# rongzhao-zhang/EfficientQ

Hardware: AMD Instinct MI355X
Metric: ptq_calibration_throughput (higher is better)
Workload: dtype i8xi8->i32 (exact) for the Gram systems and per-iteration loss convs of the layers with quantised input, f32/f64 elsewhere

## Files before the change

efficientq_amd/csrc/prox_solve.hip:

```cpp
#include "common.h"
#include "internal.h"
#include "project_dual.h"

namespace effq {

typedef float f32x16 __attribute__((ext_vector_type(16)));
typedef float f32x4 __attribute__((ext_vector_type(4)));

__global__ __launch_bounds__(256) void k_build_b(const float* __restrict__ B0, const float* __restrict__ W0,
                                                 const float* __restrict__ b0, const float* __restrict__ G,
                                                 const float* __restrict__ dual, int c2, int n, int has_bias,
                                                 float rho, float eta, float* __restrict__ Bm, int ldb, int c2p,
                                                 const float* __restrict__ wprev, float shift) {
  const size_t tot = (size_t)c2p * ldb;
  const size_t stride = (size_t)gridDim.x * blockDim.x;
  const int nw = n - has_bias;
  for (size_t e = (size_t)blockIdx.x * blockDim.x + threadIdx.x; e < tot; e += stride) {
    const int r = (int)(e / ldb), k = (int)(e % ldb);
    float v = 0.0f;
    if (r < c2 && k < n) {
      if (k < nw) {
        const size_t wi = (size_t)r * nw + k;
        v = prox_rhs(B0[(size_t)r * n + k], W0[wi], G[wi], dual[wi], eta, rho);
        if (wprev != nullptr) v = v + shift * wprev[wi];
      } else {
        v = B0[(size_t)r * n + k] + eta * b0[r];
      }
    }
    Bm[e] = v;
  }
}

__global__ __launch_bounds__(256) void k_build_b4(const float* __restrict__ B0, const float* __restrict__ W0,
                                                  const float* __restrict__ b0, const float* __restrict__ G,
                                                  const float* __restrict__ dual, int c2, int n, int has_bias,
                                                  float rho, float eta, float* __restrict__ Bm, int ldb,
                                                  const float* __restrict__ wprev, float shift) {
  __builtin_amdgcn_s_setprio(2);

  const int r = blockIdx.y;
  const int nw = n - has_bias;
  float* out = Bm + (size_t)r * ldb;
  for (int k = (blockIdx.x * blockDim.x + threadIdx.x) * 4; k < ldb; k += gridDim.x * blockDim.x * 4) {
    float4 v = make_float4(0.f, 0.f, 0.f, 0.f);
    if (r < c2 && k < nw) {
      const size_t wi = (size_t)r * nw + k;
      const float* bp = B0 + (size_t)r * n + k;
      const float4 w0 = *reinterpret_cast<const float4*>(W0 + wi), g = *reinterpret_cast<const float4*>(G + wi),
                   du = *reinterpret_cast<const float4*>(dual + wi);
      v.x = prox_rhs(bp[0], w0.x, g.x, du.x, eta, rho);
      v.y = prox_rhs(bp[1], w0.y, g.y, du.y, eta, rho);
      v.z = prox_rhs(bp[2], w0.z, g.z, du.z, eta, rho);
      v.w = prox_rhs(bp[3], w0.w, g.w, du.w, eta, rho);
      if (wprev != nullptr) {
        const float4 wp = *reinterpret_cast<const float4*>(wprev + wi);
        v.x = v.x + shift * wp.x;
        v.y = v.y + shift * wp.y;
        v.z = v.z + shift * wp.z;
        v.w = v.w + shift * wp.w;
      }
    } else if (r < c2 && k == nw && has_bias) {
      v.x = B0[(size_t)r * n + k] + eta * b0[r];
    }
    *reinterpret_cast<float4*>(out + k) = v;
  }
}

__global__ __launch_bounds__(256) void k_prox_reduce4(const float* __restrict__ part, int ldp, int nsplit, int c2, int n,
                                                      int has_bias, float* __restrict__ wstar, float* __restrict__ bstar) {
  __builtin_amdgcn_s_setprio(2);

  const int r = blockIdx.y;
  const int nw = n - has_bias;
  const size_t tot = (size_t)c2 * ldp;
  const float* row = part + (size_t)r * ldp;
  for (int k = (blockIdx.x * blockDim.x + threadIdx.x) * 4; k < ldp; k += gridDim.x * blockDim.x * 4) {
    if (k >= n) continue;
    float4 v = *reinterpret_cast<const float4*>(row + k);
    for (int z = 1; z < nsplit; ++z) {
      const float4 t = *reinterpret_cast<const float4*>(row + (size_t)z * tot + k);
      v.x += t.x;
      v.y += t.y;
      v.z += t.z;
      v.w += t.w;
    }
    if (k < nw)
      *reinterpret_cast<float4*>(wstar + (size_t)r * nw + k) = v;
    else
      bstar[r] = v.x;
  }
}

constexpr int PBK = 32, PLD = PBK + 4;

template <int MT, int WM, int WN, int NTN>
__global__ __launch_bounds__(256) void k_prox_gemm(const float* __restrict__ Bm, int ldb, const float* __restrict__ Ainv,
                                                   int lda, int n, int c2, int has_bias, float* __restrict__ wstar,
                                                   float* __restrict__ bstar, float* __restrict__ part, int ldp) {
  __builtin_amdgcn_s_setprio(2);

  constexpr int BM = 32 * MT * WM, BN = 32 * WN * NTN;
  constexpr int NA = BM * 8 / 256, NB = BN * 8 / 256;
  static_assert(WM * WN == 4 && NA >= 1 && NB >= 1, "4 waves");
  __shared__ __attribute__((aligned(16))) float As[BM * PLD];
  __shared__ __attribute__((aligned(16))) float Bs[BN * PLD];
  const int tid = threadIdx.x, lane = tid & 63, wid = tid >> 6;
  const int li = lane & 31, lh = lane >> 5;
  const int wm = wid / WN, wn = wid % WN;
  const int row0 = blockIdx.y * BM, col0 = blockIdx.x * BN;

  f32x16 acc[MT][NTN];
#pragma unroll
  for (int m = 0; m < MT; ++m)
#pragma unroll
    for (int t = 0; t < NTN; ++t)
#pragma unroll
      for (int r = 0; r < 16; ++r) acc[m][t][r] = 0.0f;

  f32x4 ra[NA], rb[NB];
  const float* pa[NA];
  const float* pb[NB];
#pragma unroll
  for (int q = 0; q < NA; ++q) {
    const int u = tid + q * 256, r = u >> 3, c4 = u & 7;
    pa[q] = Bm + (size_t)(row0 + r) * ldb + c4 * 4;
  }
#pragma unroll
  for (int q = 0; q < NB; ++q) {
    const int u = tid + q * 256, r = u >> 3, c4 = u & 7;
    pb[q] = Ainv + (size_t)min(col0 + r, n - 1) * lda + c4 * 4;
  }
#define EFFQ_PROX_FETCH(k0)                                                         \
  {                                                                                 \
    _Pragma("unroll") for (int q = 0; q < NA; ++q)                                  \
        ra[q] = *reinterpret_cast<const f32x4*>(pa[q] + (k0));                      \
    _Pragma("unroll") for (int q = 0; q < NB; ++q)                                  \
        rb[q] = *reinterpret_cast<const f32x4*>(pb[q] + (k0));                      \
  }
  const int nkt = ldb / PBK;
  const int kt0 = (int)(((long long)nkt * blockIdx.z) / gridDim.z);
  const int nk = (int)(((long long)nkt * (blockIdx.z + 1)) / gridDim.z);
  EFFQ_PROX_FETCH(kt0 * PBK)
  for (int kt = kt0; kt < nk; ++kt) {
    lds_barrier();
#pragma unroll
    for (int q = 0; q < NA; ++q) {
      const int u = tid + q * 256;
      *reinterpret_cast<f32x4*>(&As[(u >> 3) * PLD + (u & 7) * 4]) = ra[q];
    }
#pragma unroll
    for (int q = 0; q < NB; ++q) {
      const int u = tid + q * 256;
      *reinterpret_cast<f32x4*>(&Bs[(u >> 3) * PLD + (u & 7) * 4]) = rb[q];
    }
    lds_barrier();
    EFFQ_PROX_FETCH(min(kt + 1, nk - 1) * PBK)
    __builtin_amdgcn_sched_barrier(0);
#pragma unroll
    for (int q = 0; q < 4; ++q) {
      f32x4 a[MT], b[NTN];
#pragma unroll
      for (int m = 0; m < MT; ++m)
        a[m] = *reinterpret_cast<const f32x4*>(&As[((wm * MT + m) * 32 + li) * PLD + q * 8 + 4 * lh]);
#pragma unroll
      for (int t = 0; t < NTN; ++t)
        b[t] = *reinterpret_cast<const f32x4*>(&Bs[((wn * NTN + t) * 32 + li) * PLD + q * 8 + 4 * lh]);
#pragma unroll
      for (int m = 0; m < MT; ++m)
#pragma unroll
        for (int t = 0; t < NTN; ++t)
#pragma unroll
          for (int e = 0; e < 4; ++e)
            acc[m][t] = __builtin_amdgcn_mfma_f32_32x32x2f32(a[m][e], b[t][e], acc[m][t], 0, 0, 0);
    }
  }
#undef EFFQ_PROX_FETCH
  const int nw = n - has_bias;
  if (gridDim.z > 1) {
    float* P = part + (size_t)blockIdx.z * c2 * ldp;
#pragma unroll
    for (int m = 0; m < MT; ++m)
#pragma unroll
      for (int t = 0; t < NTN; ++t) {
        const int col = col0 + (wn * NTN + t) * 32 + li;
#pragma unroll
        for (int r = 0; r < 16; ++r) {
          const int row = row0 + (wm * MT + m) * 32 + (r & 3) + 8 * (r >> 2) + 4 * lh;
          if (row < c2 && col < n) P[(size_t)row * ldp + col] = acc[m][t][r];
        }
      }
    return;
  }
#pragma unroll
  for (int m = 0; m < MT; ++m)
#pragma unroll
    for (int t = 0; t < NTN; ++t) {
      const int col = col0 + (wn * NTN + t) * 32 + li;
#pragma unroll
      for (int r = 0; r < 16; ++r) {
        const int row = row0 + (wm * MT + m) * 32 + (r & 3) + 8 * (r >> 2) + 4 * lh;
        if (row < c2 && col < n) {
          if (col < nw)
            wstar[(size_t)row * nw + col] = acc[m][t][r];
          else
            bstar[row] = acc[m][t][r];
        }
      }
    }
}


typedef __bf16 bf16x8 __attribute__((ext_vector_type(8)));
typedef __bf16 bf16x4 __attribute__((ext_vector_type(4)));
constexpr int B3_K = 16;
constexpr int B3_LD = B3_K + 8;

__device__ __forceinline__ void split3(const f32x4 v, bf16x4& p0, bf16x4& p1, bf16x4& p2) {
#pragma unroll
  for (int e = 0; e < 4; ++e) {
    const __bf16 b0 = (__bf16)v[e];
    const float r1 = v[e] - (float)b0;
    const __bf16 b1 = (__bf16)r1;
    const float r2 = r1 - (float)b1;
    p0[e] = b0;
    p1[e] = b1;
    p2[e] = (__bf16)r2;
  }
}

template <int BM, int BN, int WM, int WN>
__global__ __launch_bounds__(512) void k_prox_gemm_b3(const float* __restrict__ Bm, int ldb, const float* __restrict__ Ainv,
                                                      int lda, int n, int c2, int has_bias, float* __restrict__ wstar,
                                                      float* __restrict__ bstar, float* __restrict__ part, int ldp) {
  __builtin_amdgcn_s_setprio(2);
  constexpr int MT = BM / WM / 32, NT = BN / WN / 32;
  constexpr int NA = BM * 4 / 512, NB = BN * 4 / 512;
  constexpr int STAGE = 3 * (BM + BN) * B3_LD;
  static_assert(WM * WN == 8 && MT >= 1 && NT >= 1 && NA >= 1 && NB >= 1, "8 waves");
  extern __shared__ __attribute__((aligned(16))) unsigned char b3_lds[];
  __bf16* lds = reinterpret_cast<__bf16*>(b3_lds);
  const int tid = threadIdx.x, lane = tid & 63, wid = tid >> 6;
  const int li = lane & 31, lh = lane >> 5;
  const int wm = wid / WN, wn = wid % WN;
  const int row0 = blockIdx.y * BM, col0 = blockIdx.x * BN;

// ... 101 lines not shown
          else if (col < nw)
            wstar[(size_t)row * nw + col] = acc[m][t][r];
          else
            bstar[row] = acc[m][t][r];
        }
      }
    }
}

__global__ __launch_bounds__(256) void k_prox_reduce(const float* __restrict__ part, int ldp, int nsplit, int c2, int n,
                                                     int has_bias, float* __restrict__ wstar, float* __restrict__ bstar) {
  const size_t tot = (size_t)c2 * ldp, stride = (size_t)gridDim.x * blockDim.x;
  const int nw = n - has_bias;
  for (size_t e = (size_t)blockIdx.x * blockDim.x + threadIdx.x; e < tot; e += stride) {
    const int row = (int)(e / ldp), col = (int)(e % ldp);
    if (col >= n) continue;
    float v = part[e];
    for (int z = 1; z < nsplit; ++z) v += part[(size_t)z * tot + e];
    if (col < nw)
      wstar[(size_t)row * nw + col] = v;
    else
      bstar[row] = v;
  }
}

enum ProxVariant { PROX_F32_256 = 0, PROX_F32_128 = 1, PROX_F32_64 = 2, PROX_F32_32 = 3, PROX_B3_256 = 5, PROX_B3_128 = 7 };
typedef void (*ProxGemm)(const float*, int, const float*, int, int, int, int, float*, float*, float*, int);
struct ProxTile {
  ProxVariant variant;
  int bm, bn, threads;
  size_t lds;
  ProxGemm kernel;
  hipError_t (*raise_lds)(size_t);
};
template <int MT, int WM, int WN, int NTN>
static ProxTile f32_tile(ProxVariant v) {
  return ProxTile{v, 32 * MT * WM, 32 * WN * NTN, 256, 0, k_prox_gemm<MT, WM, WN, NTN>, nullptr};
}
template <int BM, int BN, int WM, int WN>
static ProxTile b3_tile(ProxVariant v) {
  return ProxTile{v, BM, BN, 512, (size_t)2 * 3 * (BM + BN) * B3_LD * sizeof(__bf16), k_prox_gemm_b3<BM, BN, WM, WN>,
                  raise_lds_limit<k_prox_gemm_b3<BM, BN, WM, WN>>};
}
static const ProxTile TILE_F32_256 = f32_tile<2, 4, 1, 2>(PROX_F32_256);
static const ProxTile TILE_F32_128 = f32_tile<1, 4, 1, 2>(PROX_F32_128);
static const ProxTile TILE_F32_64 = f32_tile<1, 2, 2, 1>(PROX_F32_64);
static const ProxTile TILE_F32_32 = f32_tile<1, 1, 4, 1>(PROX_F32_32);
static const ProxTile TILE_B3_256 = b3_tile<256, 256, 4, 2>(PROX_B3_256);
static const ProxTile TILE_B3_128 = b3_tile<128, 128, 2, 4>(PROX_B3_128);

struct ProxPlan {
  const ProxTile* tile;
  int gx, gy, nsplit, c2p, ldb;
};
static ProxPlan prox_plan(int c2, int n) {
  ProxPlan p;
  p.c2p = (c2 > 128) ? round_up(c2, 256) : (c2 > 64) ? 128 : round_up(c2, 32);
  p.ldb = round_up(n, 32);
  const bool b3 = p.c2p >= 128 && n >= 1024;
  if (b3) p.tile = (p.c2p == 128) ? &TILE_B3_128 : &TILE_B3_256;
  else p.tile = (p.c2p >= 256) ? &TILE_F32_256 : (p.c2p == 128) ? &TILE_F32_128 : (p.c2p == 64) ? &TILE_F32_64 : &TILE_F32_32;
  p.gx = (n + p.tile->bn - 1) / p.tile->bn;
  p.gy = p.c2p / p.tile->bm;
  const int tiles = p.gx * p.gy;
  if (b3) {
    const int nkt5 = p.ldb / B3_K;
    int s5 = (256 + tiles / 2) / tiles;
    if (s5 > nkt5 / 16) s5 = nkt5 / 16;
    if (s5 < 1) s5 = 1;
    p.nsplit = s5;
    return p;
  }
  const int nkt = p.ldb / PBK;
  int s = (440 + tiles - 1) / tiles;
  if (s > nkt / 6) s = nkt / 6;
  if (s > 16) s = 16;
  if (s < 1) s = 1;
  if (p.tile == &TILE_F32_256) {
    const int smax = s > 1 ? 16 : 1;
    double best = -1.0;
    for (int c = 1; c <= smax && c <= nkt / 6; ++c) {
      const int wgs = tiles * c, rounds = (wgs + 767) / 768;
      const double score = (double)wgs / (768.0 * rounds) - 0.01 * c;
      if (score > best) { best = score; s = c; }
    }
  }
  p.nsplit = s;
  return p;
}

}

using namespace effq;

extern "C" {

int effq_prox_plan_query(int c2, int n, int* variant, int* gx, int* gy, int* nsplit) {
  EFFQ_CHECK_ARG(c2 > 0 && n > 0 && variant && gx && gy && nsplit);
  const ProxPlan p = prox_plan(c2, n);
  *variant = p.tile->variant;
  *gx = p.gx;
  *gy = p.gy;
  *nsplit = p.nsplit;
  return EFFQ_OK;
}

size_t effq_prox_ws_bytes(int c2, int n) {
  if (c2 <= 0 || n <= 0) return 0;
  const ProxPlan p = prox_plan(c2, n);
  return ((size_t)p.c2p + (p.nsplit > 1 ? (size_t)p.nsplit * c2 : 0)) * p.ldb * sizeof(float) + 256;
}

static int launch_build(const ProxSolve& s, const ProxPlan& pl, float* Bm, const float* wprev, hipStream_t st) {
  const int hb = s.has_bias ? 1 : 0;
  if (((s.n - hb) % 4) == 0) {
    const unsigned bx = (unsigned)((pl.ldb / 4 + 255) / 256);
    hipLaunchKernelGGL(k_build_b4, dim3(bx, (unsigned)pl.c2p), dim3(256), 0, st, s.B0, s.W0, s.b0, s.G, s.dual, s.c2, s.n,
                       hb, (float)s.rho, (float)s.eta, Bm, pl.ldb, wprev, (float)s.shift);
  } else {
    size_t nb = ((size_t)pl.c2p * pl.ldb + 255) / 256;
    if (nb > 4096) nb = 4096;
    hipLaunchKernelGGL(k_build_b, dim3((unsigned)nb), dim3(256), 0, st, s.B0, s.W0, s.b0, s.G, s.dual, s.c2, s.n, hb,
                       (float)s.rho, (float)s.eta, Bm, pl.ldb, pl.c2p, wprev, (float)s.shift);
  }
  EFFQ_LAUNCH_CHECK();
  return EFFQ_OK;
}

static int launch_gemm(const ProxSolve& s, const ProxPlan& pl, const float* Bm, float* part, hipStream_t st) {
  const ProxTile& t = *pl.tile;
  if (t.lds > 0) EFFQ_HIP(t.raise_lds(t.lds));
  hipLaunchKernelGGL(t.kernel, dim3(pl.gx, pl.gy, pl.nsplit), dim3(t.threads), t.lds, st, Bm, pl.ldb, s.Ainv,
                     effq_ainv_ld(s.n), s.n, s.c2, s.has_bias ? 1 : 0, s.wstar, s.bstar, part, pl.ldb);
  EFFQ_LAUNCH_CHECK();
  return EFFQ_OK;
}

static int launch_reduce(const ProxSolve& s, const ProxPlan& pl, const float* part, hipStream_t st) {
  const int hb = s.has_bias ? 1 : 0;
  if (((s.n - hb) % 4) == 0) {
    const unsigned bx = (unsigned)((pl.ldb / 4 + 255) / 256);
    hipLaunchKernelGGL(k_prox_reduce4, dim3(bx, (unsigned)s.c2), dim3(256), 0, st, part, pl.ldb, pl.nsplit, s.c2, s.n, hb,
                       s.wstar, s.bstar);
  } else {
    size_t nb = ((size_t)s.c2 * pl.ldb + 255) / 256;
    if (nb > 2048) nb = 2048;
    hipLaunchKernelGGL(k_prox_reduce, dim3((unsigned)nb), dim3(256), 0, st, part, pl.ldb, pl.nsplit, s.c2, s.n, hb,
                       s.wstar, s.bstar);
  }
  EFFQ_LAUNCH_CHECK();
  return EFFQ_OK;
}

int effq_prox_enqueue(const ProxSolve* sp, void* stream) {
  EFFQ_CHECK_ARG(sp != nullptr);
  const ProxSolve& s = *sp;
  EFFQ_CHECK_ARG(s.B0 && s.Ainv && s.W0 && s.G && s.dual && s.wstar && s.ws && s.c2 > 0 && s.n > 0 && s.nterms >= 1);
  EFFQ_CHECK_ARG(!s.has_bias || (s.b0 != nullptr && s.bstar != nullptr));
  if (s.ws_bytes < effq_prox_ws_bytes(s.c2, s.n)) {
    set_error("prox_solve: workspace %zu < required %zu", s.ws_bytes, effq_prox_ws_bytes(s.c2, s.n));
    return EFFQ_ERR_WORKSPACE;
  }
  const ProxPlan pl = prox_plan(s.c2, s.n);
  float* Bm = reinterpret_cast<float*>(s.ws);
  float* part = Bm + (size_t)pl.c2p * pl.ldb;
  hipStream_t st = as_stream(stream);
  for (int term = 0; term < s.nterms; ++term) {
    if (!(s.prebuilt && term == 0))
      if (const int rc = launch_build(s, pl, Bm, (term > 0) ? s.wstar : nullptr, st); rc != EFFQ_OK) return rc;
    if (const int rc = launch_gemm(s, pl, Bm, part, st); rc != EFFQ_OK) return rc;
    if (s.parts != nullptr)
      *s.parts = ProxParts{(pl.nsplit > 1) ? part : nullptr, pl.nsplit, pl.ldb};
    else if (pl.nsplit > 1)
      if (const int rc = launch_reduce(s, pl, part, st); rc != EFFQ_OK) return rc;
  }
  return EFFQ_OK;
}

int effq_prox_solve(const float* B0, const float* Ainv, const float* W0, const float* b0, const float* G,
                    const float* dual, int c2, int n, int has_bias, double rho, double eta, float* wstar, float* bstar,
                    void* ws, size_t ws_bytes, void* stream) {
  const ProxSolve s = {B0, Ainv, W0, b0, G, dual, c2, n, has_bias, rho, eta, 0.0, 1, false, wstar, bstar, ws, ws_bytes,
                       nullptr};
  return effq_prox_enqueue(&s, stream);
}

int effq_prox_solve_shifted(const float* B0, const float* Ainv, const float* W0, const float* b0, const float* G,
                            const float* dual, int c2, int n, int has_bias, double rho, double eta, double rho_inv,
                            int nterms, float* wstar, float* bstar, void* ws, size_t ws_bytes, void* stream) {
  EFFQ_CHECK_ARG(rho_inv >= rho && rho > 0.0 && eta >= 0.0);
  const ProxSolve s = {B0, Ainv, W0, b0, G, dual, c2, n, has_bias, rho, eta, rho_inv - rho, nterms, false, wstar, bstar,
                       ws, ws_bytes, nullptr};
  return effq_prox_enqueue(&s, stream);
}

float* effq_prox_bm(void* ws, int c2, int n, int* ldb) {
  *ldb = prox_plan(c2, n).ldb;
  return reinterpret_cast<float*>(ws);
}

}
```

efficientq_amd/csrc/spd_inverse.hip:

```cpp
#include <vector>
#include "common.h"

namespace effq {

typedef double f64x4 __attribute__((ext_vector_type(4)));

constexpr int NBK = 64;
constexpr int LDA_S = 66;
constexpr int LDB_S = 80;

__global__ __launch_bounds__(256) void k_build_a64(const float* __restrict__ A0, int n, int npad, int has_bias,
                                                   double rho, double eta, double* __restrict__ A64) {
  const size_t tot = (size_t)npad * npad;
  const size_t stride = (size_t)gridDim.x * blockDim.x;
  for (size_t e = (size_t)blockIdx.x * blockDim.x + threadIdx.x; e < tot; e += stride) {
    const int i = (int)(e / npad), j = (int)(e % npad);
    double v = 0.0;
    if (i < n && j < n) {
      v = (double)A0[(size_t)i * n + j];
      if (i == j) v += eta + ((has_bias && i == n - 1) ? 0.0 : rho);
    } else if (i == j) {
      v = 1.0;
    }
    A64[e] = v;
  }
}

__device__ __forceinline__ double readlane_f64(double v, int lane) {
  const int lo = __builtin_amdgcn_readlane(__double2loint(v), lane);
  const int hi = __builtin_amdgcn_readlane(__double2hiint(v), lane);
  return __hiloint2double(hi, lo);
}

template <int CPW>
__device__ __forceinline__ void gj_invert_regs(double (&reg)[CPW], double (*fcol)[NBK + 1], int lane, int wid) {
#pragma unroll
  for (int p = 0; p < NBK; ++p) {
    const int par = p & 1, wp = p / CPW, jp = p % CPW;
    if (wid == wp) {
      double cp = reg[0];
#pragma unroll
      for (int j = 1; j < CPW; ++j) cp = (jp == j) ? reg[j] : cp;
      fcol[par][lane] = cp;
      if (lane == p) fcol[par][NBK] = 1.0 / cp;
    }
    lds_barrier();
    const double piv = fcol[par][NBK];
    const double f = fcol[par][lane];
#pragma unroll
    for (int j = 0; j < CPW; ++j) {
      const double rp = readlane_f64(reg[j], p) * piv;
      const bool colp = (wid == wp) && (jp == j);
      double v;
      if (lane == p)
        v = colp ? piv : rp;
      else
        v = colp ? (-f * piv) : (reg[j] - f * rp);
      reg[j] = v;
    }
  }
}

constexpr int GJD_T = 1024, GJD_CPW = NBK / (GJD_T / 64);
__global__ __launch_bounds__(GJD_T) void k_gj_diag(const double* __restrict__ A, int npad, int kb,
                                                   double* __restrict__ Dinv) {
  __shared__ double fcol[2][NBK + 1];
  const int lane = threadIdx.x & 63, wid = threadIdx.x >> 6;
  double reg[GJD_CPW];
#pragma unroll
  for (int j = 0; j < GJD_CPW; ++j) reg[j] = A[(size_t)(kb + lane) * npad + kb + wid * GJD_CPW + j];
  gj_invert_regs<GJD_CPW>(reg, fcol, lane, wid);
#pragma unroll
  for (int j = 0; j < GJD_CPW; ++j) Dinv[lane * NBK + wid * GJD_CPW + j] = reg[j];
}

__device__ __forceinline__ void tile_mma64(const double* As, const double* Bs, f64x4 (&acc)[2][2]) {
  const int lane = threadIdx.x & 63, wid = threadIdx.x >> 6;
  const int wr = wid >> 1, wc = wid & 1;
  const int lr = lane & 15, lk = lane >> 4;
#pragma unroll 4
  for (int ks = 0; ks < NBK / 4; ++ks) {
    double a[2], b[2];
#pragma unroll
    for (int mi = 0; mi < 2; ++mi) a[mi] = As[(wr * 32 + mi * 16 + lr) * LDA_S + ks * 4 + lk];
#pragma unroll
    for (int ni = 0; ni < 2; ++ni) b[ni] = Bs[(ks * 4 + lk) * LDB_S + wc * 32 + ni * 16 + lr];
#pragma unroll
    for (int mi = 0; mi < 2; ++mi)
#pragma unroll
      for (int ni = 0; ni < 2; ++ni) acc[mi][ni] = __builtin_amdgcn_mfma_f64_16x16x4f64(a[mi], b[ni], acc[mi][ni], 0, 0, 0);
  }
}

__device__ __forceinline__ void load_tile(double* dst, int ld, const double* src, size_t src_ld) {
  const int tid = threadIdx.x;
  for (int e = tid; e < NBK * NBK; e += 256) {
    const int r = e >> 6, c = e & 63;
    dst[r * ld + c] = src[(size_t)r * src_ld + c];
  }
}

constexpr int GJ_CT = 4;

__global__ __launch_bounds__(256) void k_gj_panel(double* __restrict__ A, int npad, int kb,
                                                  const double* __restrict__ Dinv, double* __restrict__ NZ,
                                                  double* __restrict__ XT) {
  extern __shared__ __attribute__((aligned(16))) double sm[];
  double* As = sm;
  double* Bs = sm + NBK * LDA_S;
  const int kblk = kb / NBK;
  const int t = blockIdx.x;
  const int tid = threadIdx.x, lane = tid & 63, wid = tid >> 6;
  const int wr = wid >> 1, wc = wid & 1;
  if (t == kblk) {
    for (int e = tid; e < NBK * NBK; e += 256) A[(size_t)(kb + (e >> 6)) * npad + kb + (e & 63)] = Dinv[e];
    return;
  }
  const bool upper = t < kblk;
  const double sgn = upper ? -1.0 : 1.0;
  for (int e = tid; e < NBK * NBK; e += 256) {
    const int r = e >> 6, c = e & 63;
    const double v = upper ? A[(size_t)(t * NBK + r) * npad + kb + c] : A[(size_t)(kb + r) * npad + (size_t)t * NBK + c];
    if (upper) {
      As[r * LDA_S + c] = v;
    } else {
      As[c * LDA_S + r] = v;
    }
  }
  load_tile(Bs, LDB_S, Dinv, NBK);
  lds_barrier();
  for (int e = tid; e < NBK * NBK; e += 256) {
    const int kk = e >> 6, r = e & 63;
    XT[(size_t)kk * npad + (size_t)t * NBK + r] = sgn * As[r * LDA_S + kk];
  }
  f64x4 acc[2][2];
#pragma unroll
  for (int mi = 0; mi < 2; ++mi)
#pragma unroll
    for (int ni = 0; ni < 2; ++ni)
#pragma unroll
      for (int r = 0; r < 4; ++r) acc[mi][ni][r] = 0.0;
  tile_mma64(As, Bs, acc);
  const int lr = lane & 15, lk = lane >> 4;
#pragma unroll
  for (int mi = 0; mi < 2; ++mi)
#pragma unroll
    for (int ni = 0; ni < 2; ++ni)
#pragma unroll
      for (int r = 0; r < 4; ++r) {
        const int row = wr * 32 + mi * 16 + lk + 4 * r;
        const int col = wc * 32 + ni * 16 + lr;
        const double z = acc[mi][ni][r];
        NZ[(size_t)(t * NBK + row) * NBK + col] = -z;
        if (upper)
          A[(size_t)(t * NBK + row) * npad + kb + col] = -z;
        else
          A[(size_t)(kb + col) * npad + (size_t)t * NBK + row] = z;
      }
}

__global__ __launch_bounds__(256) void k_gj_trail_sym(double* __restrict__ A, int npad, int kb,
                                                      const double* __restrict__ NZ, const double* __restrict__ XT,
                                                      double* __restrict__ Dinv_next) {
  __shared__ __attribute__((aligned(16))) double As[NBK * LDA_S];
  __shared__ double fcol[2][NBK + 1];
  const int kblk = kb / NBK, nblk = npad / NBK;
  const int kn = kblk + 1;
  const bool ahead = Dinv_next != nullptr && kn < nblk;
  const int tid = threadIdx.x, lane = tid & 63, wid = tid >> 6;
  const int wr = wid >> 1, wc = wid & 1;
  const int lr = lane & 15, lk = lane >> 4;
  if (blockIdx.y == 0) {
    if (blockIdx.x != 0 || !ahead) return;
    for (int e = tid; e < NBK * NBK; e += 256) {
      const int r = e >> 6, c = e & 63;
      As[r * LDA_S + c] = NZ[(size_t)(kn * NBK + r) * NBK + c];
    }
    lds_barrier();
    const double* Cb = A + (size_t)(kn * NBK + wr * 32) * npad + (size_t)kn * NBK + wc * 32;
    const double* Rb = XT + (size_t)kn * NBK + wc * 32;
    f64x4 acc[2][2];
#pragma unroll
    for (int mi = 0; mi < 2; ++mi)
#pragma unroll
      for (int ni = 0; ni < 2; ++ni)
#pragma unroll
        for (int r = 0; r < 4; ++r) acc[mi][ni][r] = Cb[(size_t)(mi * 16 + lk + 4 * r) * npad + ni * 16 + lr];
#pragma unroll 4
    for (int ks = 0; ks < NBK / 4; ++ks) {
      double a[2], b[2];
#pragma unroll
      for (int mi = 0; mi < 2; ++mi) a[mi] = As[(wr * 32 + mi * 16 + lr) * LDA_S + ks * 4 + lk];
#pragma unroll
      for (int ni = 0; ni < 2; ++ni) b[ni] = Rb[(size_t)(ks * 4 + lk) * npad + ni * 16 + lr];
#pragma unroll
      for (int mi = 0; mi < 2; ++mi)
#pragma unroll
        for (int ni = 0; ni < 2; ++ni) acc[mi][ni] = __builtin_amdgcn_mfma_f64_16x16x4f64(a[mi], b[ni], acc[mi][ni], 0, 0, 0);
    }
    lds_barrier();
#pragma unroll
    for (int mi = 0; mi < 2; ++mi)
#pragma unroll
      for (int ni = 0; ni < 2; ++ni)
#pragma unroll
        for (int r = 0; r < 4; ++r)
          As[(wr * 32 + mi * 16 + lk + 4 * r) * LDA_S + wc * 32 + ni * 16 + lr] = acc[mi][ni][r];
    lds_barrier();
    constexpr int CPW = NBK / 4;
    double reg[CPW];
#pragma unroll
    for (int j = 0; j < CPW; ++j) reg[j] = As[lane * LDA_S + wid * CPW + j];
    gj_invert_regs<CPW>(reg, fcol, lane, wid);
#pragma unroll
    for (int j = 0; j < CPW; ++j) Dinv_next[lane * NBK + wid * CPW + j] = reg[j];
    return;
  }
  const int ib = (int)blockIdx.y - 1;
  if (ib == kblk) return;
  if ((int)(blockIdx.x * GJ_CT + GJ_CT - 1) < ib) return;
  for (int e = tid; e < NBK * NBK; e += 256) {
    const int r = e >> 6, c = e & 63;
    As[r * LDA_S + c] = NZ[(size_t)(ib * NBK + r) * NBK + c];
  }
  lds_barrier();
  auto live = [&](int t) -> bool {
    const int jb = blockIdx.x * GJ_CT + t;
    return t < GJ_CT && jb < nblk && jb != kblk && jb >= ib && !(ahead && ib == kn && jb == kn);
  };
  auto fetch = [&](int t, f64x4 (&c)[2][2]) {
    const int jb = blockIdx.x * GJ_CT + t;
    const double* Cb = A + (size_t)(ib * NBK + wr * 32) * npad + (size_t)jb * NBK + wc * 32;
#pragma unroll
    for (int mi = 0; mi < 2; ++mi)
#pragma unroll
      for (int ni = 0; ni < 2; ++ni)
#pragma unroll
        for (int r = 0; r < 4; ++r) c[mi][ni][r] = Cb[(size_t)(mi * 16 + lk + 4 * r) * npad + ni * 16 + lr];
  };
  f64x4 nxt[2][2];
  int t = 0;
  while (t < GJ_CT && !live(t)) ++t;
  if (t < GJ_CT) fetch(t, nxt);
  while (t < GJ_CT) {
    const int jb = blockIdx.x * GJ_CT + t;
    f64x4 acc[2][2];
#pragma unroll
    for (int mi = 0; mi < 2; ++mi)
#pragma unroll
      for (int ni = 0; ni < 2; ++ni) acc[mi][ni] = nxt[mi][ni];
    int tn = t + 1;
    while (tn < GJ_CT && !live(tn)) ++tn;
    if (tn < GJ_CT) fetch(tn, nxt);
    double* Cb = A + (size_t)(ib * NBK + wr * 32) * npad + (size_t)jb * NBK + wc * 32;
    const double* Rb = XT + (size_t)jb * NBK + wc * 32;
#pragma unroll 4
    for (int ks = 0; ks < NBK / 4; ++ks) {
      double a[2], b[2];
#pragma unroll
      for (int mi = 0; mi < 2; ++mi) a[mi] = As[(wr * 32 + mi * 16 + lr) * LDA_S + ks * 4 + lk];
#pragma unroll
      for (int ni = 0; ni < 2; ++ni) b[ni] = Rb[(size_t)(ks * 4 + lk) * npad + ni * 16 + lr];
#pragma unroll
      for (int mi = 0; mi < 2; ++mi)
#pragma unroll
        for (int ni = 0; ni < 2; ++ni) acc[mi][ni] = __builtin_amdgcn_mfma_f64_16x16x4f64(a[mi], b[ni], acc[mi][ni], 0, 0, 0);
    }
#pragma unroll
    for (int mi = 0; mi < 2; ++mi)
#pragma unroll
      for (int ni = 0; ni < 2; ++ni)
#pragma unroll
        for (int r = 0; r < 4; ++r) Cb[(size_t)(mi * 16 + lk + 4 * r) * npad + ni * 16 + lr] = acc[mi][ni][r];
    t = tn;
  }
}

__global__ __launch_bounds__(256) void k_a64_to_f32(const double* __restrict__ A64, int n, int npad,
                                                    float* __restrict__ Ainv, int lda) {
  const size_t tot = (size_t)n * lda;
  const size_t stride = (size_t)gridDim.x * blockDim.x;
  for (size_t e = (size_t)blockIdx.x * blockDim.x + threadIdx.x; e < tot; e += stride) {
    const int i = (int)(e / lda), j = (int)(e % lda);
    const int a = (i < j) ? i : j, b = (i < j) ? j : i;
    Ainv[e] = (j < n) ? (float)A64[(size_t)a * npad + b] : 0.0f;
  }
}

constexpr int WB = 4, WK = WB * NBK;
constexpr int BG_T = 128, BG_KC = 16, BG_LD = 144;
typedef double f64x2 __attribute__((ext_vector_type(2)));

struct GjBig {
  const double* Cin;
  size_t ldin;
  double* Cout;
  size_t ldout;
  int orow, ocol;
  const double* NZT;
  const double* XTW;
  size_t ldx;
  int kdim;
  int nblk;
  int i0m, j0m;
  int skip_lo, skip_hi;
  int la_lo, la_hi;
};

__global__ __launch_bounds__(256, 2) void k_gj_big(const GjBig p) {
  __shared__ __attribute__((aligned(16))) double As[2][BG_KC * BG_LD];
  __shared__ __attribute__((aligned(16))) double Bs[2][BG_KC * BG_LD];
  const int I = p.i0m + (int)blockIdx.y, J = p.j0m + (int)blockIdx.x;
  if (J < I) return;
  auto blk_live = [&](int bi, int bj) -> bool {
    if (bi > bj || bj >= p.nblk) return false;
    if ((bi >= p.skip_lo && bi < p.skip_hi) || (bj >= p.skip_lo && bj < p.skip_hi)) return false;
    if (bi >= p.la_lo && bi < p.la_hi && bj >= p.la_lo && bj < p.la_hi) return false;
    return true;
  };
  if (!(blk_live(2 * I, 2 * J) || blk_live(2 * I, 2 * J + 1) || blk_live(2 * I + 1, 2 * J) || blk_live(2 * I + 1, 2 * J + 1)))
    return;
  const int tid = threadIdx.x, lane = tid & 63, wid = tid >> 6;
  const int wr = wid >> 1, wc = wid & 1;
  const int lr = lane & 15, lk = lane >> 4;
  const int bi = 2 * I + wr, bj = 2 * J + wc;
  const bool live = blk_live(bi, bj);
  f64x4 acc[4][4];
  if (live) {
    const double* Cb = p.Cin + (size_t)bi * NBK * p.ldin + (size_t)bj * NBK;
#pragma unroll
    for (int mi = 0; mi < 4; ++mi)
#pragma unroll
      for (int ni = 0; ni < 4; ++ni)
#pragma unroll
        for (int r = 0; r < 4; ++r) acc[mi][ni][r] = Cb[(size_t)(mi * 16 + lk + 4 * r) * p.ldin + ni * 16 + lr];
  } else {
#pragma unroll
    for (int mi = 0; mi < 4; ++mi)
#pragma unroll
      for (int ni = 0; ni < 4; ++ni)
#pragma unroll
        for (int r = 0; r < 4; ++r) acc[mi][ni][r] = 0.0;
  }
  const int nch = p.kdim / BG_KC;
  if (nch > 0) {
    const int sk = tid >> 4, sc = (tid & 15) * 2;
    const double* Ag = p.NZT + (size_t)sk * p.ldx + (size_t)I * BG_T + sc;
    const double* Bg = p.XTW + (size_t)sk * p.ldx + (size_t)J * BG_T + sc;
    f64x2 ra[4], rb[4];
#pragma unroll
    for (int v = 0; v < 4; ++v) {
      ra[v] = *reinterpret_cast<const f64x2*>(Ag + v * 32);
      rb[v] = *reinterpret_cast<const f64x2*>(Bg + v * 32);
    }
#pragma unroll
    for (int v = 0; v < 4; ++v) {
      *reinterpret_cast<f64x2*>(&As[0][sk * BG_LD + sc + v * 32]) = ra[v];
      *reinterpret_cast<f64x2*>(&Bs[0][sk * BG_LD + sc + v * 32]) = rb[v];
    }
    lds_barrier();
    for (int c = 0; c < nch; ++c) {
      const int buf = c & 1;
      if (c + 1 < nch) {
        const size_t off = (size_t)(c + 1) * BG_KC * p.ldx;
#pragma unroll
        for (int v = 0; v < 4; ++v) {
          ra[v] = *reinterpret_cast<const f64x2*>(Ag + off + v * 32);
          rb[v] = *reinterpret_cast<const f64x2*>(Bg + off + v * 32);
        }
      }
      if (live) {
#pragma unroll
        for (int ks = 0; ks < BG_KC / 4; ++ks) {
          double a[4], b[4];
#pragma unroll
          for (int mi = 0; mi < 4; ++mi) a[mi] = As[buf][(ks * 4 + lk) * BG_LD + wr * 64 + mi * 16 + lr];
#pragma unroll
          for (int ni = 0; ni < 4; ++ni) b[ni] = Bs[buf][(ks * 4 + lk) * BG_LD + wc * 64 + ni * 16 + lr];
#pragma unroll
          for (int mi = 0; mi < 4; ++mi)
#pragma unroll
            for (int ni = 0; ni < 4; ++ni)
              acc[mi][ni] = __builtin_amdgcn_mfma_f64_16x16x4f64(a[mi], b[ni], acc[mi][ni], 0, 0, 0);
        }
      }
      if (c + 1 < nch) {
#pragma unroll
        for (int v = 0; v < 4; ++v) {
          *reinterpret_cast<f64x2*>(&As[buf ^ 1][sk * BG_LD + sc + v * 32]) = ra[v];
          *reinterpret_cast<f64x2*>(&Bs[buf ^ 1][sk * BG_LD + sc + v * 32]) = rb[v];
        }
      }
      lds_barrier();
    }
  }
  if (live) {
    double* Ob = p.Cout + ((size_t)bi * NBK - p.orow) * p.ldout + ((size_t)bj * NBK - p.ocol);
#pragma unroll
    for (int mi = 0; mi < 4; ++mi)
#pragma unroll
      for (int ni = 0; ni < 4; ++ni)
#pragma unroll
        for (int r = 0; r < 4; ++r) Ob[(size_t)(mi * 16 + lk + 4 * r) * p.ldout + ni * 16 + lr] = acc[mi][ni][r];
  }
}

__global__ __launch_bounds__(256) void k_gj_panel_w(const double* __restrict__ A, int npad, int kb0, int m,
                                                    const double* __restrict__ Dw, double* __restrict__ NZT,
                                                    double* __restrict__ XTW, size_t ldx) {
  extern __shared__ __attribute__((aligned(16))) double sm[];
  double* As = sm;
  double* Bs = sm + NBK * LDA_S;
  const int t = blockIdx.x, c = blockIdx.y;
  if (t >= kb0 && t < kb0 + m) return;
  const int tid = threadIdx.x, lane = tid & 63, wid = tid >> 6;
  const int wr = wid >> 1, wc = wid & 1;
  const bool upper = t < kb0;
  const double sgn = upper ? -1.0 : 1.0;
  const int ldd = m * NBK;
  f64x4 acc[2][2];
#pragma unroll
  for (int mi = 0; mi < 2; ++mi)
#pragma unroll
    for (int ni = 0; ni < 2; ++ni)
#pragma unroll
      for (int r = 0; r < 4; ++r) acc[mi][ni][r] = 0.0;
  for (int a = 0; a < m; ++a) {
    for (int e = tid; e < NBK * NBK; e += 256) {
      const int r = e >> 6, cc = e & 63;
      if (upper)
        As[r * LDA_S + cc] = A[(size_t)(t * NBK + r) * npad + (size_t)(kb0 + a) * NBK + cc];
      else
        As[cc * LDA_S + r] = A[(size_t)((kb0 + a) * NBK + r) * npad + (size_t)t * NBK + cc];
    }
    load_tile(Bs, LDB_S, Dw + (size_t)a * NBK * ldd + (size_t)c * NBK, (size_t)ldd);
    lds_barrier();
    if (a == c)
      for (int e = tid; e < NBK * NBK; e += 256) {
        const int kk = e >> 6, r = e & 63;
        XTW[(size_t)(c * NBK + kk) * ldx + (size_t)t * NBK + r] = sgn * As[r * LDA_S + kk];
      }
    tile_mma64(As, Bs, acc);
    lds_barrier();
  }
  const int lr = lane & 15, lk = lane >> 4;
#pragma unroll
  for (int mi = 0; mi < 2; ++mi)
#pragma unroll
    for (int ni = 0; ni < 2; ++ni)
#pragma unroll
      for (int r = 0; r < 4; ++r)
        As[(wr * 32 + mi * 16 + lk + 4 * r) * LDA_S + wc * 32 + ni * 16 + lr] = acc[mi][ni][r];
  lds_barrier();
  for (int e = tid; e < NBK * NBK; e += 256) {
    const int kk = e >> 6, r = e & 63;
    NZT[(size_t)(c * NBK + kk) * ldx + (size_t)t * NBK + r] = -As[r * LDA_S + kk];
  }
}

__global__ __launch_bounds__(256) void k_gj_wback_w(double* __restrict__ A, int npad, int kb0, int m,
                                                    const double* __restrict__ Dw, const double* __restrict__ NZT,
                                                    size_t ldx) {
  __shared__ double Ts[NBK * (NBK + 1)];
  const int t = blockIdx.x, c = blockIdx.y, tid = threadIdx.x;
  const int ldd = m * NBK;
  if (t >= kb0 && t < kb0 + m) {
    const int a = t - kb0;
    if (a > c) return;
    for (int e = tid; e < NBK * NBK; e += 256) {
      const int r = e >> 6, cc = e & 63;
      A[(size_t)(t * NBK + r) * npad + (size_t)(kb0 + c) * NBK + cc] = Dw[(size_t)(a * NBK + r) * ldd + (size_t)c * NBK + cc];
    }
    return;
  }
  if (t < kb0) {
    for (int e = tid; e < NBK * NBK; e += 256) {
      const int kk = e >> 6, r = e & 63;
      Ts[kk * (NBK + 1) + r] = NZT[(size_t)(c * NBK + kk) * ldx + (size_t)t * NBK + r];
    }
    __syncthreads();
    for (int e = tid; e < NBK * NBK; e += 256) {
      const int r = e >> 6, kk = e & 63;
      A[(size_t)(t * NBK + r) * npad + (size_t)(kb0 + c) * NBK + kk] = Ts[kk * (NBK + 1) + r];
    }
  } else {
    for (int e = tid; e < NBK * NBK; e += 256) {
      const int kk = e >> 6, r = e & 63;
      A[(size_t)((kb0 + c) * NBK + kk) * npad + (size_t)t * NBK + r] = -NZT[(size_t)(c * NBK + kk) * ldx + (size_t)t * NBK + r];
    }
  }
}

__global__ __launch_bounds__(256) void k_mirror_blocks(double* __restrict__ D, int nd) {
  const size_t tot = (size_t)nd * nd;
  for (size_t e = (size_t)blockIdx.x * blockDim.x + threadIdx.x; e < tot; e += (size_t)gridDim.x * blockDim.x) {
    const int i = (int)(e / nd), j = (int)(e % nd);
    if ((i / NBK) > (j / NBK)) D[e] = D[(size_t)j * nd + i];
  }
}

}

using namespace effq;

extern "C" {

static size_t gj64_aux_doubles(size_t npad) { return 2 * (size_t)NBK * npad + 2 * NBK * NBK; }

constexpr int GJ_WIDE_MIN_BLOCKS = 100;
static bool gj_takes_wide(int nblk) { return nblk >= GJ_WIDE_MIN_BLOCKS; }

size_t effq_spd_inverse_ws_bytes(int n) {
  if (n <= 0) return 0;
  const size_t npad = (size_t)round_up(n, NBK);
  size_t d = npad * npad + gj64_aux_doubles(npad);
  if (gj_takes_wide((int)(npad / NBK))) {
    const size_t ldx = (size_t)round_up((int)npad, BG_T);
    d = npad * npad + 2 * (size_t)WK * ldx + (size_t)WK * WK + gj64_aux_doubles(WK);
  }
  return d * sizeof(double) + 256;
}

int effq_ainv_ld(int n) { return n > 0 ? round_up(n, 32) : 0; }

static int gj64_sweep(double* A64, int npad, double* aux, hipStream_t st) {
  const int nblk = npad / NBK;
  double* XT = aux;
  double* NZ = XT + (size_t)NBK * npad;
  double* Dinv = NZ + (size_t)NBK * npad;
  const size_t lds = (size_t)(NBK * LDA_S + NBK * LDB_S) * sizeof(double);
  for (int k = 0; k < nblk; ++k) {
    const int kb = k * NBK;
    double* Dk = Dinv + (size_t)(k & 1) * NBK * NBK;
    double* Dn = Dinv + (size_t)((k + 1) & 1) * NBK * NBK;
    if (k == 0) hipLaunchKernelGGL(k_gj_diag, dim3(1), dim3(GJD_T), 0, st, A64, npad, kb, Dk);
    hipLaunchKernelGGL(k_gj_panel, dim3(nblk), dim3(256), lds, st, A64, npad, kb, Dk, NZ, XT);
    if (nblk > 1)
      hipLaunchKernelGGL(k_gj_trail_sym, dim3((nblk + GJ_CT - 1) / GJ_CT, nblk + 1), dim3(256), 0, st, A64, npad, kb, NZ,
                         XT, Dn);
    EFFQ_LAUNCH_CHECK();
  }
  return EFFQ_OK;
}

struct GjWideCtx {
  int dev;
  hipStream_t caller, helper;
  hipEvent_t e1, e2;
};
static thread_local std::vector<GjWideCtx> g_gj_ctx;

static int gj_wide_ctx(hipStream_t caller, GjWideCtx** out) {
  int dev = 0;
  EFFQ_HIP(hipGetDevice(&dev));
  for (GjWideCtx& c : g_gj_ctx)
    if (c.dev == dev && c.caller == caller) {
      *out = &c;
      return EFFQ_OK;
    }
  GjWideCtx c;
  c.dev = dev;
  c.caller = caller;
  int prio = 0;
  if (hipStreamGetPriority(caller, &prio) != hipSuccess) prio = 0;
  EFFQ_HIP(hipStreamCreateWithPriority(&c.helper, hipStreamNonBlocking, prio));
  EFFQ_HIP(hipEventCreateWithFlags(&c.e1, hipEventDisableTiming));
  EFFQ_HIP(hipEventCreateWithFlags(&c.e2, hipEventDisableTiming));
  g_gj_ctx.push_back(c);
  *out = &g_gj_ctx.back();
  return EFFQ_OK;
}

static int gj_wide_sweep(double* A64, int npad, double* aux, hipStream_t st) {
  const int nblk = npad / NBK;
  const size_t ldx = (size_t)round_up(npad, BG_T);
  double* NZT = aux;
  double* XTW = NZT + (size_t)WK * ldx;
  double* Dw = XTW + (size_t)WK * ldx;
  double* aux64 = Dw + (size_t)WK * WK;
  const int nK = (nblk + WB - 1) / WB, nm = (nblk + 1) / 2;
  GjWideCtx* ctx = nullptr;
  if (nK > 1) {
    const int rc = gj_wide_ctx(st, &ctx);
    if (rc != EFFQ_OK) return rc;
  }
  hipStream_t s2 = ctx ? ctx->helper : st;
  const size_t lds = (size_t)(NBK * LDA_S + NBK * LDB_S) * sizeof(double);
  auto pivot_block = [&](int k0, int mk, int kdim, hipStream_t s) -> int {
    GjBig g;
    memset(&g, 0, sizeof(g));
    g.Cin = A64; g.ldin = (size_t)npad;
    g.Cout = Dw; g.ldout = (size_t)mk * NBK; g.orow = k0 * NBK; g.ocol = k0 * NBK;
    g.NZT = NZT; g.XTW = XTW; g.ldx = ldx; g.kdim = kdim; g.nblk = nblk;
    g.i0m = k0 / 2; g.j0m = k0 / 2;
    g.skip_lo = g.skip_hi = -1; g.la_lo = g.la_hi = -1;
    const int span = (mk + 1) / 2;
    hipLaunchKernelGGL(k_gj_big, dim3(span, span), dim3(256), 0, s, g);
    EFFQ_LAUNCH_CHECK();
    const int rc = gj64_sweep(Dw, mk * NBK, aux64, s);
    if (rc != EFFQ_OK) return rc;
    hipLaunchKernelGGL(k_mirror_blocks, dim3(64), dim3(256), 0, s, Dw, mk * NBK);
    EFFQ_LAUNCH_CHECK();
    return EFFQ_OK;
  };
  {
    const int rc = pivot_block(0, nblk < WB ? nblk : WB, 0, st);
    if (rc != EFFQ_OK) return rc;
  }
  for (int K = 0; K < nK; ++K) {
    const int kb0 = K * WB, m = (nblk - kb0 < WB) ? nblk - kb0 : WB;
    const int kn0 = kb0 + WB, mn = (K + 1 < nK) ? ((nblk - kn0 < WB) ? nblk - kn0 : WB) : 0;
    hipLaunchKernelGGL(k_gj_panel_w, dim3(nblk, m), dim3(256), lds, st, A64, npad, kb0, m, Dw, NZT, XTW, ldx);
    EFFQ_LAUNCH_CHECK();
    if (ctx) {
      EFFQ_HIP(hipEventRecord(ctx->e1, st));
      EFFQ_HIP(hipStreamWaitEvent(s2, ctx->e1, 0));
    }
    hipLaunchKernelGGL(k_gj_wback_w, dim3(nblk, m), dim3(256), 0, s2, A64, npad, kb0, m, Dw, NZT, ldx);
    EFFQ_LAUNCH_CHECK();
    if (mn > 0) {
      const int rc = pivot_block(kn0, mn, m * NBK, s2);
      if (rc != EFFQ_OK) return rc;
    }
    if (nblk > m) {
      GjBig g;
      memset(&g, 0, sizeof(g));
      g.Cin = A64; g.ldin = (size_t)npad;
      g.Cout = A64; g.ldout = (size_t)npad; g.orow = 0; g.ocol = 0;
      g.NZT = NZT; g.XTW = XTW; g.ldx = ldx; g.kdim = m * NBK; g.nblk = nblk;
      g.i0m = 0; g.j0m = 0;
      g.skip_lo = kb0; g.skip_hi = kb0 + m;
      g.la_lo = mn > 0 ? kn0 : -1; g.la_hi = mn > 0 ? kn0 + mn : -1;
      hipLaunchKernelGGL(k_gj_big, dim3(nm, nm), dim3(256), 0, st, g);
      EFFQ_LAUNCH_CHECK();
    }
    if (ctx) {
      EFFQ_HIP(hipEventRecord(ctx->e2, s2));
      EFFQ_HIP(hipStreamWaitEvent(st, ctx->e2, 0));
    }
  }
  return EFFQ_OK;
}

int effq_spd_inverse_prepare(void* stream) {
  GjWideCtx* ctx = nullptr;
  return gj_wide_ctx(as_stream(stream), &ctx);
}

int effq_spd_inverse(const float* A0, int n, int has_bias, double rho, double eta, float* Ainv, void* ws,
                     size_t ws_bytes, void* stream) {
  EFFQ_CHECK_ARG(A0 && Ainv && ws && n > 0);
  EFFQ_CHECK_ARG(eta > 0.0 && rho >= 0.0);
  if (ws_bytes < effq_spd_inverse_ws_bytes(n)) {
    set_error("spd_inverse: workspace %zu < required %zu", ws_bytes, effq_spd_inverse_ws_bytes(n));
    return EFFQ_ERR_WORKSPACE;
  }
  const int npad = round_up(n, NBK);
  double* A64 = reinterpret_cast<double*>(ws);
  double* aux = A64 + (size_t)npad * npad;
  hipStream_t st = as_stream(stream);
  {
    size_t nb = ((size_t)npad * npad + 255) / 256;
    if (nb > 8192) nb = 8192;
    hipLaunchKernelGGL(k_build_a64, dim3((unsigned)nb), dim3(256), 0, st, A0, n, npad, has_bias, rho, eta, A64);
    EFFQ_LAUNCH_CHECK();
  }
  const size_t lds = (size_t)(NBK * LDA_S + NBK * LDB_S) * sizeof(double);
  EFFQ_HIP(raise_lds_limit<k_gj_panel>(lds));
  EFFQ_HIP(raise_lds_limit<k_gj_panel_w>(lds));
  const int rc = gj_takes_wide(npad / NBK) ? gj_wide_sweep(A64, npad, aux, st) : gj64_sweep(A64, npad, aux, st);
  if (rc != EFFQ_OK) return rc;
  {
    const int lda = effq_ainv_ld(n);
    size_t nb = ((size_t)n * lda + 255) / 256;
    if (nb > 8192) nb = 8192;
    hipLaunchKernelGGL(k_a64_to_f32, dim3((unsigned)nb), dim3(256), 0, st, A64, n, npad, Ainv, lda);
    EFFQ_LAUNCH_CHECK();
  }
  return EFFQ_OK;
}

int effq_spd_inverse_plan(int n, int* wide, int* nblk, int* pivot_blocks) {
  EFFQ_CHECK_ARG(n > 0 && wide && nblk && pivot_blocks);
  const int nb = round_up(n, NBK) / NBK;
  *wide = gj_takes_wide(nb) ? 1 : 0;
  *nblk = nb;
  *pivot_blocks = *wide ? (nb + WB - 1) / WB : nb;
  return EFFQ_OK;
}

}
// ... 1 lines not shown
```

Baseline: 25.60.

## Fuse shifted-term reduce into RHS build; widen GJ trailing update workgroups

In the shifted prox solve, the split-K partial reduction for intermediate terms is folded into the next term's RHS build. This removes one kernel launch and one write/read round trip of wstar per term. Separately, the Gauss-Jordan trailing update now runs one wave group per column tile (GJ_CT groups per workgroup) in parallel, instead of looping serially over tiles with a prefetch. Each group preloads its whole XT panel into registers. The added register pressure and larger workgroups may reduce occupancy.

Measured after the change: 25.75 (median of 6 runs). Within noise of the previous version (+0.6%).

```diff
diff --git a/efficientq_amd/csrc/prox_solve.hip b/efficientq_amd/csrc/prox_solve.hip
--- a/efficientq_amd/csrc/prox_solve.hip
+++ b/efficientq_amd/csrc/prox_solve.hip
@@ -91,6 +91,43 @@
   }
 }
 
+__global__ __launch_bounds__(256) void k_prox_reduce_build4(const float* __restrict__ part, int ldp, int nsplit, int c2,
+                                                            const float* __restrict__ B0, const float* __restrict__ W0,
+                                                            const float* __restrict__ G, const float* __restrict__ dual,
+                                                            int n, int has_bias, float rho, float eta, float shift,
+                                                            float* __restrict__ Bm) {
+  __builtin_amdgcn_s_setprio(2);
+
+  const int r = blockIdx.y;
+  const int nw = n - has_bias;
+  const size_t tot = (size_t)c2 * ldp;
+  const float* row = part + (size_t)r * ldp;
+  for (int k = (blockIdx.x * blockDim.x + threadIdx.x) * 4; k < nw; k += gridDim.x * blockDim.x * 4) {
+    float4 wp = *reinterpret_cast<const float4*>(row + k);
+    for (int z = 1; z < nsplit; ++z) {
+      const float4 t = *reinterpret_cast<const float4*>(row + (size_t)z * tot + k);
+      wp.x += t.x;
+      wp.y += t.y;
+      wp.z += t.z;
+      wp.w += t.w;
+    }
+    const size_t wi = (size_t)r * nw + k;
+    const float* bp = B0 + (size_t)r * n + k;
+    const float4 w0 = *reinterpret_cast<const float4*>(W0 + wi), g = *reinterpret_cast<const float4*>(G + wi),
+                 du = *reinterpret_cast<const float4*>(dual + wi);
+    float4 v;
+    v.x = prox_rhs(bp[0], w0.x, g.x, du.x, eta, rho);
+    v.y = prox_rhs(bp[1], w0.y, g.y, du.y, eta, rho);
+    v.z = prox_rhs(bp[2], w0.z, g.z, du.z, eta, rho);
+    v.w = prox_rhs(bp[3], w0.w, g.w, du.w, eta, rho);
+    v.x = v.x + shift * wp.x;
+    v.y = v.y + shift * wp.y;
+    v.z = v.z + shift * wp.z;
+    v.w = v.w + shift * wp.w;
+    *reinterpret_cast<float4*>(Bm + (size_t)r * ldp + k) = v;
+  }
+}
+
 constexpr int PBK = 32, PLD = PBK + 4;
 
 template <int MT, int WM, int WN, int NTN>
@@ -498,6 +535,15 @@
   return EFFQ_OK;
 }
 
+static int launch_reduce_build(const ProxSolve& s, const ProxPlan& pl, const float* part, float* Bm, hipStream_t st) {
+  const int hb = s.has_bias ? 1 : 0;
+  const unsigned bx = (unsigned)(((s.n - hb) / 4 + 255) / 256);
+  hipLaunchKernelGGL(k_prox_reduce_build4, dim3(bx, (unsigned)s.c2), dim3(256), 0, st, part, pl.ldb, pl.nsplit, s.c2, s.B0,
+                     s.W0, s.G, s.dual, s.n, hb, (float)s.rho, (float)s.eta, (float)s.shift, Bm);
+  EFFQ_LAUNCH_CHECK();
+  return EFFQ_OK;
+}
+
 int effq_prox_enqueue(const ProxSolve* sp, void* stream) {
   EFFQ_CHECK_ARG(sp != nullptr);
   const ProxSolve& s = *sp;
@@ -511,13 +557,18 @@
   float* Bm = reinterpret_cast<float*>(s.ws);
   float* part = Bm + (size_t)pl.c2p * pl.ldb;
   hipStream_t st = as_stream(stream);
+  const int nwrow = s.n - (s.has_bias ? 1 : 0);
+  const bool fuse_terms = pl.nsplit > 1 && s.parts == nullptr && nwrow > 0 && (nwrow % 4) == 0;
   for (int term = 0; term < s.nterms; ++term) {
-    if (!(s.prebuilt && term == 0))
+    if (term > 0 && fuse_terms) {
+      if (const int rc = launch_reduce_build(s, pl, part, Bm, st); rc != EFFQ_OK) return rc;
+    } else if (!(s.prebuilt && term == 0)) {
       if (const int rc = launch_build(s, pl, Bm, (term > 0) ? s.wstar : nullptr, st); rc != EFFQ_OK) return rc;
+    }
     if (const int rc = launch_gemm(s, pl, Bm, part, st); rc != EFFQ_OK) return rc;
     if (s.parts != nullptr)
       *s.parts = ProxParts{(pl.nsplit > 1) ? part : nullptr, pl.nsplit, pl.ldb};
-    else if (pl.nsplit > 1)
+    else if (pl.nsplit > 1 && !(fuse_terms && term + 1 < s.nterms))
       if (const int rc = launch_reduce(s, pl, part, st); rc != EFFQ_OK) return rc;
   }
   return EFFQ_OK;
diff --git a/efficientq_amd/csrc/spd_inverse.hip b/efficientq_amd/csrc/spd_inverse.hip
--- a/efficientq_amd/csrc/spd_inverse.hip
+++ b/efficientq_amd/csrc/spd_inverse.hip
@@ -159,46 +159,76 @@
       }
 }
 
-__global__ __launch_bounds__(256) void k_gj_trail_sym(double* __restrict__ A, int npad, int kb,
-                                                      const double* __restrict__ NZ, const double* __restrict__ XT,
-                                                      double* __restrict__ Dinv_next) {
+constexpr int GJT_T = 256 * GJ_CT;
+static_assert(GJT_T == GJD_T, "the look-ahead workgroup inverts with k_gj_diag's mapping");
+__global__ __launch_bounds__(GJT_T) void k_gj_trail_sym(double* __restrict__ A, int npad, int kb,
+                                                        const double* __restrict__ NZ, const double* __restrict__ XT,
+                                                        double* __restrict__ Dinv_next) {
   __shared__ __attribute__((aligned(16))) double As[NBK * LDA_S];
   __shared__ double fcol[2][NBK + 1];
   const int kblk = kb / NBK, nblk = npad / NBK;
   const int kn = kblk + 1;
   const bool ahead = Dinv_next != nullptr && kn < nblk;
   const int tid = threadIdx.x, lane = tid & 63, wid = tid >> 6;
-  const int wr = wid >> 1, wc = wid & 1;
+  const int grp = wid >> 2, wr = (wid >> 1) & 1, wc = wid & 1;
   const int lr = lane & 15, lk = lane >> 4;
-  if (blockIdx.y == 0) {
-    if (blockIdx.x != 0 || !ahead) return;
-    for (int e = tid; e < NBK * NBK; e += 256) {
-      const int r = e >> 6, c = e & 63;
-      As[r * LDA_S + c] = NZ[(size_t)(kn * NBK + r) * NBK + c];
-    }
-    lds_barrier();
-    const double* Cb = A + (size_t)(kn * NBK + wr * 32) * npad + (size_t)kn * NBK + wc * 32;
-    const double* Rb = XT + (size_t)kn * NBK + wc * 32;
-    f64x4 acc[2][2];
+  const bool la = blockIdx.y == 0;
+  if (la && (blockIdx.x != 0 || !ahead)) return;
+  const int ib = la ? kn : (int)blockIdx.y - 1;
+  if (!la && (ib == kblk || (int)(blockIdx.x * GJ_CT + GJ_CT - 1) < ib)) return;
+  const int jb = la ? kn : (int)blockIdx.x * GJ_CT + grp;
+  const bool live = la ? (grp == 0) : (jb < nblk && jb != kblk && jb >= ib && !(ahead && ib == kn && jb == kn));
+  double z[NBK * NBK / GJT_T];
+#pragma unroll
+  for (int q = 0; q < NBK * NBK / GJT_T; ++q) z[q] = NZ[(size_t)ib * NBK * NBK + tid + q * GJT_T];
+  double* Cb = A + (size_t)(ib * NBK + wr * 32) * npad + (size_t)jb * NBK + wc * 32;
+  f64x4 acc[2][2];
+  double bq[NBK / 4][2];
+  if (live) {
+    const double* Rb = XT + (size_t)jb * NBK + wc * 32;
 #pragma unroll
     for (int mi = 0; mi < 2; ++mi)
 #pragma unroll
       for (int ni = 0; ni < 2; ++ni)
 #pragma unroll
         for (int r = 0; r < 4; ++r) acc[mi][ni][r] = Cb[(size_t)(mi * 16 + lk + 4 * r) * npad + ni * 16 + lr];
-#pragma unroll 4
+#pragma unroll
+    for (int ks = 0; ks < NBK / 4; ++ks)
+#pragma unroll
+      for (int ni = 0; ni < 2; ++ni) bq[ks][ni] = Rb[(size_t)(ks * 4 + lk) * npad + ni * 16 + lr];
+  }
+#pragma unroll
+  for (int q = 0; q < NBK * NBK / GJT_T; ++q) {
+    const int e = tid + q * GJT_T;
+    As[(e >> 6) * LDA_S + (e & 63)] = z[q];
+  }
+  lds_barrier();
+  if (live) {
+#pragma unroll
     for (int ks = 0; ks < NBK / 4; ++ks) {
-      double a[2], b[2];
+      double a[2];
 #pragma unroll
       for (int mi = 0; mi < 2; ++mi) a[mi] = As[(wr * 32 + mi * 16 + lr) * LDA_S + ks * 4 + lk];
 #pragma unroll
-      for (int ni = 0; ni < 2; ++ni) b[ni] = Rb[(size_t)(ks * 4 + lk) * npad + ni * 16 + lr];
-#pragma unroll
       for (int mi = 0; mi < 2; ++mi)
 #pragma unroll
-        for (int ni = 0; ni < 2; ++ni) acc[mi][ni] = __builtin_amdgcn_mfma_f64_16x16x4f64(a[mi], b[ni], acc[mi][ni], 0, 0, 0);
-    }
-    lds_barrier();
+        for (int ni = 0; ni < 2; ++ni)
+          acc[mi][ni] = __builtin_amdgcn_mfma_f64_16x16x4f64(a[mi], bq[ks][ni], acc[mi][ni], 0, 0, 0);
+    }
+  }
+  if (!la) {
+    if (live) {
+#pragma unroll
+      for (int mi = 0; mi < 2; ++mi)
+#pragma unroll
+        for (int ni = 0; ni < 2; ++ni)
+#pragma unroll
+          for (int r = 0; r < 4; ++r) Cb[(size_t)(mi * 16 + lk + 4 * r) * npad + ni * 16 + lr] = acc[mi][ni][r];
+    }
+    return;
+  }
+  lds_barrier();
+  if (live) {
 #pragma unroll
     for (int mi = 0; mi < 2; ++mi)
 #pragma unroll
@@ -206,74 +236,14 @@
 #pragma unroll
         for (int r = 0; r < 4; ++r)
           As[(wr * 32 + mi * 16 + lk + 4 * r) * LDA_S + wc * 32 + ni * 16 + lr] = acc[mi][ni][r];
-    lds_barrier();
-    constexpr int CPW = NBK / 4;
-    double reg[CPW];
-#pragma unroll
-    for (int j = 0; j < CPW; ++j) reg[j] = As[lane * LDA_S + wid * CPW + j];
-    gj_invert_regs<CPW>(reg, fcol, lane, wid);
-#pragma unroll
-    for (int j = 0; j < CPW; ++j) Dinv_next[lane * NBK + wid * CPW + j] = reg[j];
-    return;
-  }
-  const int ib = (int)blockIdx.y - 1;
-  if (ib == kblk) return;
-  if ((int)(blockIdx.x * GJ_CT + GJ_CT - 1) < ib) return;
-  for (int e = tid; e < NBK * NBK; e += 256) {
-    const int r = e >> 6, c = e & 63;
-    As[r * LDA_S + c] = NZ[(size_t)(ib * NBK + r) * NBK + c];
   }
   lds_barrier();
-  auto live = [&](int t) -> bool {
-    const int jb = blockIdx.x * GJ_CT + t;
-    return t < GJ_CT && jb < nblk && jb != kblk && jb >= ib && !(ahead && ib == kn && jb == kn);
-  };
-  auto fetch = [&](int t, f64x4 (&c)[2][2]) {
-    const int jb = blockIdx.x * GJ_CT + t;
-    const double* Cb = A + (size_t)(ib * NBK + wr * 32) * npad + (size_t)jb * NBK + wc * 32;
-#pragma unroll
-    for (int mi = 0; mi < 2; ++mi)
-#pragma unroll
-      for (int ni = 0; ni < 2; ++ni)
-#pragma unroll
-        for (int r = 0; r < 4; ++r) c[mi][ni][r] = Cb[(size_t)(mi * 16 + lk + 4 * r) * npad + ni * 16 + lr];
-  };
-  f64x4 nxt[2][2];
-  int t = 0;
-  while (t < GJ_CT && !live(t)) ++t;
-  if (t < GJ_CT) fetch(t, nxt);
-  while (t < GJ_CT) {
-    const int jb = blockIdx.x * GJ_CT + t;
-    f64x4 acc[2][2];
-#pragma unroll
-    for (int mi = 0; mi < 2; ++mi)
-#pragma unroll
-      for (int ni = 0; ni < 2; ++ni) acc[mi][ni] = nxt[mi][ni];
-    int tn = t + 1;
-    while (tn < GJ_CT && !live(tn)) ++tn;
-    if (tn < GJ_CT) fetch(tn, nxt);
-    double* Cb = A + (size_t)(ib * NBK + wr * 32) * npad + (size_t)jb * NBK + wc * 32;
-    const double* Rb = XT + (size_t)jb * NBK + wc * 32;
-#pragma unroll 4
-    for (int ks = 0; ks < NBK / 4; ++ks) {
-      double a[2], b[2];
-#pragma unroll
-      for (int mi = 0; mi < 2; ++mi) a[mi] = As[(wr * 32 + mi * 16 + lr) * LDA_S + ks * 4 + lk];
-#pragma unroll
-      for (int ni = 0; ni < 2; ++ni) b[ni] = Rb[(size_t)(ks * 4 + lk) * npad + ni * 16 + lr];
-#pragma unroll
-      for (int mi = 0; mi < 2; ++mi)
-#pragma unroll
-        for (int ni = 0; ni < 2; ++ni) acc[mi][ni] = __builtin_amdgcn_mfma_f64_16x16x4f64(a[mi], b[ni], acc[mi][ni], 0, 0, 0);
-    }
-#pragma unroll
-    for (int mi = 0; mi < 2; ++mi)
-#pragma unroll
-      for (int ni = 0; ni < 2; ++ni)
-#pragma unroll
-        for (int r = 0; r < 4; ++r) Cb[(size_t)(mi * 16 + lk + 4 * r) * npad + ni * 16 + lr] = acc[mi][ni][r];
-    t = tn;
-  }
+  double reg[GJD_CPW];
+#pragma unroll
+  for (int j = 0; j < GJD_CPW; ++j) reg[j] = As[lane * LDA_S + wid * GJD_CPW + j];
+  gj_invert_regs<GJD_CPW>(reg, fcol, lane, wid);
+#pragma unroll
+  for (int j = 0; j < GJD_CPW; ++j) Dinv_next[lane * NBK + wid * GJD_CPW + j] = reg[j];
 }
 
 __global__ __launch_bounds__(256) void k_a64_to_f32(const double* __restrict__ A64, int n, int npad,
@@ -536,7 +506,7 @@
     if (k == 0) hipLaunchKernelGGL(k_gj_diag, dim3(1), dim3(GJD_T), 0, st, A64, npad, kb, Dk);
     hipLaunchKernelGGL(k_gj_panel, dim3(nblk), dim3(256), lds, st, A64, npad, kb, Dk, NZ, XT);
     if (nblk > 1)
-      hipLaunchKernelGGL(k_gj_trail_sym, dim3((nblk + GJ_CT - 1) / GJ_CT, nblk + 1), dim3(256), 0, st, A64, npad, kb, NZ,
+      hipLaunchKernelGGL(k_gj_trail_sym, dim3((nblk + GJ_CT - 1) / GJ_CT, nblk + 1), dim3(GJT_T), 0, st, A64, npad, kb, NZ,
                          XT, Dn);
     EFFQ_LAUNCH_CHECK();
   }
```
